# kolenyo2099/revers-o

Hardware: AMD Instinct MI355X
Metric: images/sec embed+top-k (PE-L14-336, 1M x 1024 gallery) (higher is better)
Workload: dtype bf16

## Files before the change

include/revo.h:

```cpp
#ifndef REVO_H
#define REVO_H
#include <stdint.h>

#ifdef __cplusplus
extern "C" {
#endif

typedef struct revo_vit revo_vit;
typedef struct revo_gallery revo_gallery;

typedef struct revo_vit_cfg {
    int32_t image_size, patch_size, width, layers, heads, mlp_dim, out_dim, pool_heads;
    int32_t use_cls;
    int32_t use_ls;
    float ln_eps, rope_theta;
    int32_t pool_mlp_dim;
} revo_vit_cfg;

typedef struct revo_tensor {
    const char* name;
    const float* data;
    int64_t numel;
} revo_tensor;

// ... 62 lines not shown
int32_t revo_search_estimates(int32_t k);
int32_t revo_search_plan(const revo_gallery* g, int32_t n_queries, int32_t k, int64_t* out4);
int32_t revo_search_candidates(revo_gallery* g, const float* queries, int32_t n_queries, int32_t k, int32_t top_m,
                               uint32_t* bounds, void* stream);
int32_t revo_search_finish(revo_gallery* g, int32_t n_queries, int32_t k, int32_t has_threshold, float threshold,
                           int64_t index_offset, const uint32_t* all_bounds, int32_t parts, int32_t top_m, float* scores,
                           int64_t* indices, int32_t* counts, float* cert, void* stream);
int32_t revo_search_exact(revo_gallery* g, int32_t n, const int32_t* q_idx, const float* need, int32_t k,
                          int32_t has_threshold, float threshold, int64_t index_offset, float* scores, int64_t* indices,
                          int32_t* counts, void* stream);
int32_t revo_search_stats(revo_gallery* g, int32_t* out8, void* stream);
int32_t revo_topk_merge(const float* scores, const int64_t* indices, int32_t parts, int32_t n_queries, int32_t k,
                        int32_t has_threshold, float threshold, float* out_scores, int64_t* out_indices,
                        int32_t* out_counts, void* stream);

int64_t revo_topk_packed_bytes(int32_t n_queries, int32_t k);
int32_t revo_topk_merge_packed(const void* packed, int32_t parts, int32_t n_queries, int32_t k, int32_t has_threshold,
                               float threshold, float* out_scores, int64_t* out_indices, int32_t* out_counts,
                               int32_t* unc_count, int32_t* unc_q, float* unc_need, void* stream);

int32_t revo_op_gemm(int32_t epilogue, const void* a_bf16, int64_t lda, const void* b_bf16, int64_t ldb, int32_t m,
                     int32_t n, int32_t k, void* c, int64_t ldc, const float* bias, const float* gamma, void* stream);
int32_t revo_op_gemm_rope(const void* a_bf16, int64_t lda, const void* b_bf16, int64_t ldb, int32_t m, int32_t n, int32_t k,
                          void* c_bf16, int64_t ldc, const float* bias, const float* cos_sin, int32_t seq,
                          int32_t head_dim, int32_t rope_cols, void* stream);
int32_t revo_op_gemm_resid_ln(const void* a_bf16, int64_t lda, const void* b_bf16, int64_t ldb, int32_t m, int32_t n, int32_t k,
                              float* c, int64_t ldc, const float* bias, const float* gamma, void* xb_bf16, int64_t ldxb,
                              void* stats, int32_t* done, void* xlo_bf16, int32_t x_in_planes, int32_t planes_out, void* stream);
int32_t revo_op_gemm_ln_in(int32_t epilogue, const void* a_bf16, int64_t lda, const void* b_bf16, int64_t ldb, int32_t m, int32_t n,
                           int32_t k, void* c_bf16, int64_t ldc, const float* bias, const float* csum, const void* stats,
                           int32_t parts, float eps, void* tele, void* stream);
int32_t revo_op_gemm_ln_in_rope(const void* a_bf16, int64_t lda, const void* b_bf16, int64_t ldb, int32_t m, int32_t n, int32_t k,
                                void* c_bf16, int64_t ldc, const float* bias, const float* csum, const void* stats, int32_t parts,
                                float eps, const float* cos_sin, int32_t seq, int32_t head_dim, int32_t rope_cols, void* stream);
int32_t revo_op_gemm_resid_norm(const void* a_bf16, int64_t lda, const void* b_bf16, int64_t ldb, int32_t m, int32_t n, int32_t k,
                                float* c, int64_t ldc, const float* bias, const float* gamma, void* ln_out_bf16, int64_t ln_ldo,
                                float eps, int32_t* fused, void* stream);
int32_t revo_probe_mfma(const void* src_bf16, int64_t n_elems, float* sink, int32_t blocks, int32_t iters, void* stream);
int64_t revo_probe_mfma_flops(int32_t blocks, int32_t iters);
int32_t revo_probe_copy(void* dst, const void* src, int64_t bytes, void* stream);
#ifdef REVO_EXPERIMENTS
int32_t revo_vit_set_debug_layers(revo_vit* vit, int32_t n_layers);
int32_t revo_vit_read_residual(revo_vit* vit, int32_t batch, float* dst, void* stream);
int32_t revo_vit_read_tap(revo_vit* vit, int32_t which, int32_t batch, void* dst, void* stream);
int32_t revo_search_set_mode(revo_gallery* g, int32_t mode);
int32_t revo_debug_set_remove_chunk(int64_t rows);
int32_t revo_op_set_phase_groups(int32_t groups);
int32_t revo_op_set_qstores(int32_t on);
int32_t revo_debug_gemm_stamps(void* buf, int32_t items);
int32_t revo_debug_attention_clock(void* buf);
int32_t revo_debug_gemm_forms(int32_t reset);
int32_t revo_op_set_gemm_tile(int32_t tile);
int32_t revo_op_set_variant(int32_t flags);
int32_t revo_op_set_ln_fold(int32_t on);
int32_t revo_op_set_gemm_debug(int32_t flags);
int64_t revo_debug_scan_plan(int32_t Q, int64_t rows, int64_t* out, int32_t cap);
int32_t revo_debug_stream_in_planes(const revo_vit* vit, int32_t batch);
int64_t revo_debug_read_workspace(revo_gallery* g, int64_t offset, int64_t bytes, void* host_dst);
int32_t revo_debug_seed_bounds(revo_gallery* g, const uint32_t* bounds);
int32_t revo_probe_gridbar(int32_t mode, void* ctr_err, void* buf, int32_t n16, int32_t blocks, int32_t threads,
                           int32_t iters, float* sink, void* stamps, void* stream);
int32_t revo_debug_scan_stats(int64_t* out8);
#endif
int32_t revo_op_layernorm(const float* x, int64_t ldx, const float* w, const float* b, float eps, int32_t rows,
                          int32_t width, void* out, int64_t ldo, int32_t out_is_bf16, void* stream);
int32_t revo_op_layernorm_logits(const float* x, int64_t ldx, const float* w, const float* b, float eps, int32_t rows,
                                 int32_t width, float* out, int64_t ldo, const float* qk, const float* ck, int32_t heads,
                                 int32_t seq, float* logits, void* stream);
int32_t revo_op_linear_f32(int32_t epi, const float* A, int64_t lda, const float* Wt, int64_t ldw, const float* bias, int32_t M,
                           int32_t N, int32_t K, float* C, int64_t ldc, void* stream);
int32_t revo_op_pool_rows(const float* x, int64_t ldx, const float* logits, int32_t batch, int32_t seq, int32_t width,
                          int32_t heads, float* u, void* stream);
int32_t revo_op_rope(void* qkv_bf16, int64_t ld, const float* cos_sin, int32_t rows, int32_t seq, int32_t width,
                     int32_t heads, void* stream);
int32_t revo_op_attention(const void* qkv_bf16, int64_t ld, void* out_bf16, int64_t ldo, int32_t batch, int32_t seq,
                          int32_t heads, int32_t head_dim, void* stream);
int32_t revo_op_f32_to_bf16(const float* src, int64_t ld_src, void* dst_bf16, int64_t ld_dst, int64_t rows,
                            int32_t cols, void* stream);

int32_t revo_prof_enable(int32_t on);
int32_t revo_prof_reset(void);
int32_t revo_prof_report(char* buf, int32_t capacity);

typedef struct revo_crop_job {
    const uint8_t* src;
    int32_t height, width;
    int64_t row_stride;
    int32_t x0, y0, x1, y1;
} revo_crop_job;
int32_t revo_preprocess_crop_resize(const revo_crop_job* jobs, int32_t n, int32_t out_size, uint8_t* out, void* stream);

#ifdef __cplusplus
}
#endif
#endif
```

revers-o_amd/_lib.py:

```python
import ctypes as C
import os

_HERE = os.path.dirname(os.path.abspath(__file__))
LIB_PATH = os.path.join(_HERE, "librevo.so")


class RevoError(RuntimeError):
    pass


class VitCfg(C.Structure):
    _fields_ = [(n, C.c_int32) for n in (
        "image_size", "patch_size", "width", "layers", "heads", "mlp_dim", "out_dim", "pool_heads",
        "use_cls", "use_ls")] + [("ln_eps", C.c_float), ("rope_theta", C.c_float), ("pool_mlp_dim", C.c_int32)]


class Tensor(C.Structure):
    _fields_ = [("name", C.c_char_p), ("data", C.c_void_p), ("numel", C.c_int64)]


class CropJob(C.Structure):
    _fields_ = [("src", C.c_void_p), ("height", C.c_int32), ("width", C.c_int32), ("row_stride", C.c_int64),
                ("x0", C.c_int32), ("y0", C.c_int32), ("x1", C.c_int32), ("y1", C.c_int32)]

# ... 29 lines not shown
    "revo_search_mmr": (_i32, [_p, _p, _i32, _i32, _i32, _f32, _i32, _f32, _i64, _p, _p, _p, _p, _p]),
    "revo_search_topk": (_i32, [_p, _p, _i32, _i32, _i32, _f32, _i64, _p, _p, _p, _p]),
    "revo_search_topk_large": (_i32, [_p, _p, _i32, _i32, _i32, _f32, _i64, _p, _p, _p, _p]),
    "revo_search_ksel": (_i32, [_i32]),
    "revo_search_set_total_rows": (_i32, [_p, _i64]),
    "revo_search_set_filter": (_i32, [_p, _p, _i64, _i32, _p]),
    "revo_search_set_groups": (_i32, [_p, _p, _i64, _i32, _p]),
    "revo_search_groups": (_i32, [_p, _p, _i32, _i32, _i32, _i32, _f32, _i64, _p, _p, _p, _p, _p, _p]),
    "revo_search_estimates": (_i32, [_i32]),
    "revo_search_plan": (_i32, [_p, _i32, _i32, C.POINTER(C.c_int64)]),
    "revo_search_candidates": (_i32, [_p, _p, _i32, _i32, _i32, _p, _p]),
    "revo_search_finish": (_i32, [_p, _i32, _i32, _i32, _f32, _i64, _p, _i32, _i32, _p, _p, _p, _p, _p]),
    "revo_search_exact": (_i32, [_p, _i32, _p, _p, _i32, _i32, _f32, _i64, _p, _p, _p, _p]),
    "revo_search_stats": (_i32, [_p, C.POINTER(C.c_int32), _p]),
    "revo_topk_merge": (_i32, [_p, _p, _i32, _i32, _i32, _i32, _f32, _p, _p, _p, _p]),
    "revo_topk_packed_bytes": (_i64, [_i32, _i32]),
    "revo_topk_merge_packed": (_i32, [_p, _i32, _i32, _i32, _i32, _f32, _p, _p, _p, _p, _p, _p, _p]),
    "revo_op_gemm": (_i32, [_i32, _p, _i64, _p, _i64, _i32, _i32, _i32, _p, _i64, _p, _p, _p]),
    "revo_op_gemm_resid_ln": (_i32, [_p, _i64, _p, _i64, _i32, _i32, _i32, _p, _i64, _p, _p, _p, _i64, _p, C.POINTER(C.c_int32), _p, _i32,
                                     _i32, _p]),
    "revo_op_gemm_ln_in": (_i32, [_i32, _p, _i64, _p, _i64, _i32, _i32, _i32, _p, _i64, _p, _p, _p, _i32, _f32, _p, _p]),
    "revo_op_gemm_rope": (_i32, [_p, _i64, _p, _i64, _i32, _i32, _i32, _p, _i64, _p, _p, _i32, _i32, _i32, _p]),
    "revo_op_gemm_ln_in_rope": (_i32, [_p, _i64, _p, _i64, _i32, _i32, _i32, _p, _i64, _p, _p, _p, _i32, _f32, _p, _i32, _i32, _i32,
                                       _p]),
    "revo_op_gemm_resid_norm": (_i32, [_p, _i64, _p, _i64, _i32, _i32, _i32, _p, _i64, _p, _p, _p, _i64, _f32, C.POINTER(C.c_int32),
                                       _p]),
    "revo_op_layernorm": (_i32, [_p, _i64, _p, _p, _f32, _i32, _i32, _p, _i64, _i32, _p]),
    "revo_op_layernorm_logits": (_i32, [_p, _i64, _p, _p, _f32, _i32, _i32, _p, _i64, _p, _p, _i32, _i32, _p, _p]),
    "revo_op_linear_f32": (_i32, [_i32, _p, _i64, _p, _i64, _p, _i32, _i32, _i32, _p, _i64, _p]),
    "revo_op_pool_rows": (_i32, [_p, _i64, _p, _i32, _i32, _i32, _i32, _p, _p]),
    "revo_op_rope": (_i32, [_p, _i64, _p, _i32, _i32, _i32, _i32, _p]),
    "revo_op_attention": (_i32, [_p, _i64, _p, _i64, _i32, _i32, _i32, _i32, _p]),
    "revo_op_f32_to_bf16": (_i32, [_p, _i64, _p, _i64, _i64, _i32, _p]),
    "revo_prof_enable": (_i32, [_i32]),
    "revo_prof_reset": (_i32, []),
    "revo_prof_report": (_i32, [C.c_char_p, _i32]),
    "revo_preprocess_crop_resize": (_i32, [C.POINTER(CropJob), _i32, _i32, _p, _p]),
    "revo_probe_mfma": (_i32, [_p, _i64, _p, _i32, _i32, _p]),
    "revo_probe_mfma_flops": (_i64, [_i32, _i32]),
    "revo_probe_copy": (_i32, [_p, _p, _i64, _p]),
}

EXPERIMENT_SIGNATURES = {
    "revo_vit_set_debug_layers": (_i32, [_p, _i32]),
    "revo_vit_read_residual": (_i32, [_p, _i32, _p, _p]),
    "revo_vit_read_tap": (_i32, [_p, _i32, _i32, _p, _p]),
    "revo_search_set_mode": (_i32, [_p, _i32]),
    "revo_op_set_gemm_tile": (_i32, [_i32]),
    "revo_op_set_phase_groups": (_i32, [_i32]),
    "revo_op_set_qstores": (_i32, [_i32]),
    "revo_debug_gemm_forms": (_i32, [_i32]),
    "revo_debug_gemm_stamps": (_i32, [_p, _i32]),
    "revo_debug_attention_clock": (_i32, [_p]),
    "revo_op_set_variant": (_i32, [_i32]),
    "revo_op_set_ln_fold": (_i32, [_i32]),
    "revo_op_set_gemm_debug": (_i32, [_i32]),
    "revo_debug_scan_stats": (_i32, [C.POINTER(C.c_int64)]),
    "revo_debug_set_remove_chunk": (_i32, [_i64]),
    "revo_debug_seed_bounds": (_i32, [_p, _p]),
    "revo_debug_read_workspace": (_i64, [_p, _i64, _i64, _p]),
    "revo_debug_stream_in_planes": (_i32, [_p, _i32]),
    "revo_probe_gridbar": (_i32, [_i32, _p, _p, _i32, _i32, _i32, _i32, _p, _p, _p]),
    "revo_debug_scan_plan": (_i64, [_i32, _i64, C.POINTER(C.c_int64), _i32]),
}
BASE_SIGNATURES = dict(SIGNATURES)
if os.environ.get("REVO_LIBRARY_PATH"):
    LIB_PATH = os.environ["REVO_LIBRARY_PATH"]
elif os.environ.get("REVO_EXPERIMENTS") == "1":
    LIB_PATH = os.path.join(_HERE, "librevo_exp.so")
if os.environ.get("REVO_EXPERIMENTS") == "1":
    SIGNATURES = dict(SIGNATURES, **EXPERIMENT_SIGNATURES)

_lib = None
_lib_exp = None


def product_is_experiment_build():
    return os.environ.get("REVO_EXPERIMENTS") == "1"


def load_exp():
    global _lib_exp
    if _lib_exp is not None:
        return _lib_exp
    import torch
    path = os.path.join(_HERE, "librevo_exp.so")
    if not os.path.exists(path):
        raise RevoError(f"{path} not found: build it with `make -C revers-o_amd/csrc exp`")
    lib = C.CDLL(path)
    for name, (res, args) in dict(BASE_SIGNATURES, **EXPERIMENT_SIGNATURES).items():
        fn = getattr(lib, name)
        fn.restype = res
        fn.argtypes = args
    _lib_exp = lib
    return lib


def load():
    global _lib
    if _lib is not None:
        return _lib
    import torch
    if not os.path.exists(LIB_PATH):
        raise RevoError(
            f"{LIB_PATH} not found: build it with `python -c 'import __graft_entry__ as g; g.build()'` "
            "(or `make -C revers-o_amd/csrc`).  There is no CPU fallback for the hot path.")
# ... 30 lines not shown
```

revers-o_amd/csrc/api.hip:

```cpp
#include <algorithm>
#include <cmath>
#include <cstdlib>
#include <cstring>
#include <map>
#include <memory>
#include <mutex>
#include <string>
#include <vector>

#include "../../include/revo.h"
#include "api_internal.h"
#include "kernels.h"

static thread_local std::string g_err;
void revo_set_error(const std::string& msg) { g_err = msg; }
extern "C" const char* revo_last_error(void) { return g_err.c_str(); }
extern "C" int32_t revo_version(void) { return 100; }

extern "C" int32_t revo_sync(void* stream) {
    REVO_HIP_CHECK(hipStreamSynchronize((hipStream_t)stream));
    return 0;
}

namespace {
// ... 637 lines not shown
}
extern "C" int32_t revo_op_gemm_rope(const void* a, int64_t lda, const void* b, int64_t ldb, int32_t m, int32_t n,
                                     int32_t k, void* c, int64_t ldc, const float* bias, const float* cos_sin,
                                     int32_t seq, int32_t head_dim, int32_t rope_cols, void* stream) {
    API_BEGIN
    revo::GemmArgs g{};
    g.A = (const bf16_t*)a; g.lda = lda; g.B = (const bf16_t*)b; g.ldb = ldb; g.M = m; g.N = n; g.K = k; g.C = c; g.ldc = ldc;
    g.bias = bias; g.rope_cs = (const float2*)cos_sin; g.rope_S = seq; g.rope_hd = head_dim; g.rope_cols = rope_cols;
    return revo::launch_gemm(revo::EPI_BF16_ROPE, g, (hipStream_t)stream);
    API_END
}
extern "C" int32_t revo_op_gemm_ln_in_rope(const void* a, int64_t lda, const void* b, int64_t ldb, int32_t m, int32_t n, int32_t k,
                                           void* c, int64_t ldc, const float* bias, const float* csum, const void* stats,
                                           int32_t parts, float eps, const float* cos_sin, int32_t seq, int32_t head_dim,
                                           int32_t rope_cols, void* stream) {
    API_BEGIN
    REVO_REQUIRE(a && b && c && csum && stats && cos_sin, "op_gemm_ln_in_rope: null argument");
    revo::GemmArgs g{};
    g.A = (const bf16_t*)a; g.lda = lda; g.B = (const bf16_t*)b; g.ldb = ldb; g.M = m; g.N = n; g.K = k; g.C = c; g.ldc = ldc;
    g.bias = bias; g.rope_cs = (const float2*)cos_sin; g.rope_S = seq; g.rope_hd = head_dim; g.rope_cols = rope_cols;
    g.lnc_stats = (const float2*)stats; g.lnc_parts = parts; g.lnc_c = csum; g.lnc_eps = eps;
    return revo::launch_gemm(revo::EPI_BF16_ROPE, g, (hipStream_t)stream);
    API_END
}
extern "C" int32_t revo_op_gemm_resid_norm(const void* a, int64_t lda, const void* b, int64_t ldb, int32_t m, int32_t n, int32_t k,
                                           float* c, int64_t ldc, const float* bias, const float* gamma, void* ln_out,
                                           int64_t ln_ldo, float eps, int32_t* fused, void* stream) {
    API_BEGIN
    REVO_REQUIRE(a && b && c && ln_out && fused, "op_gemm_resid_norm: null argument");
    constexpr long OP_WS_ELEMS = 16l << 20;
    hipStream_t st = (hipStream_t)stream;
    float* ws = nullptr;
    REVO_HIP_CHECK(hipMallocAsync((void**)&ws, OP_WS_ELEMS * 4, st));
    int flag = 0;
    const LnAfter ln{eps, (bf16_t*)ln_out, ln_ldo, &flag, nullptr, nullptr, nullptr, 0, 0};
    const int rc = gemm("gemm_op", revo::EPI_RESID_F32, (const bf16_t*)a, lda, (const bf16_t*)b, ldb, m, n, k, c, ldc, bias, gamma,
                        st, ws, OP_WS_ELEMS, &ln);
    REVO_HIP_CHECK(hipFreeAsync(ws, st));
    *fused = flag;
    return rc;
    API_END
}
#ifdef REVO_EXPERIMENTS
extern "C" int32_t revo_op_set_variant(int32_t flags) {
    revo::gemm_force_gy((flags >> 4) & 15);
    revo::attention_force_nw((flags >> 8) & 15);
    revo::gemm_set_tail_split(((flags >> 12) & 1) ? 0 : 1);
    revo::gemm_set_persistent(((flags >> 16) & 1) ? 0 : 1);
    revo::gemm_set_splitk(((flags >> 17) & 1) ? 0 : 1);
    revo::gemm_set_min_tiles256(((flags >> 18) & 1) ? 0 : 100);
    revo::gemm_set_ring(((flags >> 19) & 1) ? 0 : 1, 0);
    revo::gemm_set_rows192(((flags >> 3) & 1) ? 0 : 1);
    revo::attention_set_shape16((flags >> 20) & 1);
    return 0;
}
extern "C" int32_t revo_op_set_ln_fold(int32_t on) {
    REVO_REQUIRE(on >= 0 && on <= 2, "set_ln_fold: 0 (LayerNorm kernels), 1 (folded, stream in planes: default) or 2 (folded, fp32 stream + bf16 copy)");
    revo::gemm_set_ln_fold(on);
    return 0;
}
extern "C" int32_t revo_op_set_qstores(int32_t on) {
    revo::gemm_set_qstores(on);
    return 0;
}
extern "C" int32_t revo_op_set_phase_groups(int32_t groups) {
    REVO_REQUIRE(groups >= 0 && groups <= 4, "set_phase_groups: 0 (heuristic), 1 (off) or 2..4");
    revo::gemm_set_phase_groups(groups);
    return 0;
}
extern "C" int32_t revo_debug_attention_clock(void* buf) {
    revo::attention_set_clock_buffer((unsigned long long*)buf);
    return 0;
}
extern "C" int32_t revo_debug_gemm_stamps(void* buf, int32_t items) {
    revo::gemm_set_stamps((unsigned long long*)buf, buf ? items : 0);
    return 0;
}
extern "C" int32_t revo_debug_gemm_forms(int32_t reset) { return (int32_t)revo::gemm_debug_forms(reset); }
extern "C" int32_t revo_op_set_gemm_tile(int32_t tile) {
    REVO_REQUIRE(tile == 0 || tile == 128 || tile == 256, "set_gemm_tile: 0, 128 or 256");
    revo::gemm_force_tile(tile);
    return 0;
}
extern "C" int32_t revo_op_set_gemm_debug(int32_t flags) {
    revo::gemm_set_debug(flags & 3);
    revo::gemm_set_stagger(((flags >> 28) & 15) * 200, 2 + ((flags >> 2) & 3));
    revo::topk_scan256_set_debug(((flags >> 13) & 7) | (((flags >> 20) & 255) << 3));
    return revo_op_set_variant(flags);
}
extern "C" int64_t revo_debug_scan_plan(int32_t Q, int64_t rows, int64_t* out, int32_t cap) {
    if (Q < 1 || rows < 1 || !out || cap < 2) return -1;
    return (int64_t)revo::topk_scan256_plan_dump(Q, (long)rows, (long*)out, cap);
}
extern "C" int32_t revo_debug_stream_in_planes(const revo_vit* v, int32_t batch) {
    if (!v || !v->xlo) return 0;
    const int W = v->cfg.width, Md = v->cfg.mlp_dim, rows = batch * v->S;
    return revo::gemm_ln_planes_enabled() && revo::gemm_resid_folds(rows, W, W, W, W, W) && revo::gemm_resid_folds(rows, W, Md, Md, Md, W);
}
#endif
extern "C" int32_t revo_op_layernorm(const float* x, int64_t ldx, const float* w, const float* b, float eps,
                                     int32_t rows, int32_t width, void* out, int64_t ldo, int32_t out_is_bf16,
                                     void* stream) {
    API_BEGIN
    return revo::launch_layernorm(x, ldx, w, b, eps, rows, width, out, ldo, out_is_bf16, (hipStream_t)stream);
    API_END
}
extern "C" int32_t revo_op_layernorm_logits(const float* x, int64_t ldx, const float* w, const float* b, float eps, int32_t rows,
// ... 43 lines not shown
```

revers-o_amd/csrc/attention.hip:

```cpp
#include "kernels.h"
#include <type_traits>

namespace revo {

template <int OFF>
__device__ __forceinline__ uint64_t att_tr_read(uint32_t lds_addr) {
    uint64_t v;
    asm volatile("ds_read_b64_tr_b16 %0, %1 offset:%2" : "=v"(v) : "v"(lds_addr), "n"(OFF));
    return v;
}
template <int ROWB, int DB, int OFF0>
__device__ __forceinline__ void att_v_issue(uint64_t (&v)[2][DB][2], const uint32_t (&va)[DB]) {
#define ATT_V1(S2, D)                                                          \
    v[S2][D][0] = att_tr_read<OFF0 + (16 * S2) * ROWB>(va[D]);                 \
    v[S2][D][1] = att_tr_read<OFF0 + (16 * S2 + 8) * ROWB>(va[D]);
    ATT_V1(0, 0) ATT_V1(0, 1)
    if constexpr (DB == 3) { ATT_V1(0, 2) }
    ATT_V1(1, 0) ATT_V1(1, 1)
    if constexpr (DB == 3) { ATT_V1(1, 2) }
#undef ATT_V1
}
template <int DB, int LEFT = 0>
__device__ __forceinline__ void att_v_wait(uint64_t (&v)[2][DB][2]) {
    if constexpr (DB == 2) {
        asm volatile("s_waitcnt lgkmcnt(%8)"
                     : "+v"(v[0][0][0]), "+v"(v[0][0][1]), "+v"(v[0][1][0]), "+v"(v[0][1][1]), "+v"(v[1][0][0]),
                       "+v"(v[1][0][1]), "+v"(v[1][1][0]), "+v"(v[1][1][1])
                     : "n"(LEFT));
    } else {
        asm volatile("s_waitcnt lgkmcnt(%12)"
                     : "+v"(v[0][0][0]), "+v"(v[0][0][1]), "+v"(v[0][1][0]), "+v"(v[0][1][1]), "+v"(v[0][2][0]),
                       "+v"(v[0][2][1]), "+v"(v[1][0][0]), "+v"(v[1][0][1]), "+v"(v[1][1][0]), "+v"(v[1][1][1]),
                       "+v"(v[1][2][0]), "+v"(v[1][2][1])
                     : "n"(LEFT));
    }
}
typedef uint32_t att_u32x4 __attribute__((ext_vector_type(4)));
template <int OFF>
__device__ __forceinline__ att_u32x4 att_read_b128(uint32_t lds_addr) {
    att_u32x4 v;
    asm volatile("ds_read_b128 %0, %1 offset:%2" : "=v"(v) : "v"(lds_addr), "n"(OFF));
    return v;
}
template <int LEFT>
__device__ __forceinline__ void att_k_wait(att_u32x4& k) {
    asm volatile("s_waitcnt lgkmcnt(%1)" : "+v"(k) : "n"(LEFT));
}
__device__ __forceinline__ bf16x8 att_v_frag(uint64_t lo, uint64_t hi) {
    typedef uint64_t u64x2 __attribute__((ext_vector_type(2)));
    const u64x2 c = {lo, hi};
    return __builtin_bit_cast(bf16x8, c);
}

struct AttDmaSrc {
    __amdgpu_buffer_rsrc_t rsrc;
};
__device__ __forceinline__ void att_dma_init(AttDmaSrc& src, const void* base, int bytes) {
    src.rsrc = __builtin_amdgcn_make_buffer_rsrc((void*)base, 0, bytes, 0x00020000);
}
__device__ __forceinline__ void att_dma_issue(const AttDmaSrc& src, char* dst, uint32_t voff, uint32_t soff) {
    __builtin_amdgcn_raw_ptr_buffer_load_lds(src.rsrc, (__attribute__((address_space(3))) void*)dst, 16, voff, soff, 0, 0);
}

template <int HD, int NW, int DBG = 0, bool STAG = false>
__global__ __launch_bounds__(NW * 64, (HD == 64 && NW >= 6) ? 4 : 1) void attn_fwd_kernel(const bf16_t* __restrict__ qkv, long ld,
                                                          bf16_t* __restrict__ out, long ldo, int S, int H, float c,
                                                          int q_rot, int k_lo
#ifdef REVO_EXPERIMENTS
                                                          , unsigned long long* clk
#endif
                                                          ) {
    static_assert(HD == 64 || HD == 96, "body attention kernel is built for head_dim 64 (B16, L14) and 96 (G14)");
#ifdef REVO_EXPERIMENTS
    unsigned long long clk_t0 = 0, clk_r0 = 0;
    if (clk) { clk_t0 = __builtin_amdgcn_s_memtime(); clk_r0 = __builtin_amdgcn_s_memrealtime(); }
#endif
    constexpr int dbg = DBG;
    constexpr int KS = HD / 16;
    constexpr int DB = HD / 32;
    constexpr int CH = HD / 8;
    constexpr int ROWB = HD == 64 ? 128 : 256;
    constexpr int TILE = 64 * ROWB;
    constexpr int BUF = 2 * TILE;
    static_assert(!STAG || (HD == 64 && NW == 8), "");
    constexpr int LOOK = HD == 64 ? 2 : 1;
    constexpr int NBUF = LOOK + 1 + (STAG ? 1 : 0);
    constexpr int NI = BUF / 1024;
    constexpr int NPW = (NI + NW - 1) / NW;
    constexpr int NDUMMY = NPW * NW - NI;
    constexpr int LPR = ROWB / 16;
    constexpr int RPI = 64 / LPR;
    __shared__ __attribute__((aligned(16))) char lds[NBUF * BUF + NDUMMY * 1024];

    const int tid = threadIdx.x;
    const int wave = __builtin_amdgcn_readfirstlane(tid >> 6), lane = tid & 63;
    const int r = lane & 31, hh = lane >> 5;
    int bh, qblk;
    {
        const int nq = gridDim.x, nbh = gridDim.y, L = blockIdx.y * nq + blockIdx.x;
        const int full = (nbh / 8) * 8;
        if (L < full * nq) {
            const int xcd = L & 7, slot = L >> 3;
            bh = (slot / nq) * 8 + xcd;
            qblk = slot % nq;
        } else {
            const int r = L - full * nq;
            bh = full + r / nq;
            qblk = r % nq;
        }
    }
    const int b = bh / H, h = bh - b * H;
    const int W = H * HD;
    const long rowbase = (long)b * S;
    const int q0 = qblk * (NW * 32) + wave * 32;
    const bool wave_active = q0 < S;
    const bool row_valid = q0 + r < S;
    const int qpos = row_valid ? q0 + r : S - 1;
    const int qrow = q_rot ? (qpos + 1 < S ? qpos + 1 : 0) : qpos;
    const int qrow_c = qrow;

    const bf16_t* kg = qkv + W + h * HD;
    const bf16_t* vg = qkv + 2 * W + h * HD;

    bf16x8 qf[KS];
    {
        const bf16_t* qp = qkv + (rowbase + qrow_c) * ld + h * HD + 8 * hh;
#pragma unroll
        for (int ks = 0; ks < KS; ++ks) qf[ks] = *(const bf16x8*)(qp + 16 * ks);
    }

    const int nkeys = S - k_lo;
    const int nt = (nkeys + 63) / 64;
    AttDmaSrc dma_src;
    att_dma_init(dma_src, kg + (rowbase + k_lo) * ld, (int)(((long)(nkeys - 1) * ld + W + HD) * 2));
    uint32_t dma_voff[NPW];
#pragma unroll
    for (int i = 0; i < NPW; ++i) {
        const int j = wave + NW * i;
        const int row = j * RPI + lane / LPR;
        const int cp = lane % LPR;
        const int isv = row >= 64, key = row & 63;
        const int swz = HD == 64 ? (isv ? (((key >> 1) & 1) << 2) : ((key >> 1) & 7))
                                 : (isv ? ((key & 3) << 2) : (key & 15));
        const int ch = cp ^ swz;
        dma_voff[i] = (ch < CH && j < NI) ? (uint32_t)(((long)key * ld + (isv ? W : 0)) * 2 + ch * 16) : 0x80000000u;
// ... 165 lines not shown
            ps2 = (f32x2){1.f, 1.f};
            _Pragma("unroll") for (int kb_ = 0; kb_ < 2; ++kb_)
                _Pragma("unroll") for (int j_ = 0; j_ < 8; ++j_) pw[kb_][j_] = pack_bf16x2(sacc[kb_][2 * j_], sacc[kb_][2 * j_ + 1]);
        }
        float ps = ps2.x + ps2.y;
        if (!__all(ps < 0x1p80f)) {
            asm volatile("" ::: "memory");
            scores();
            float mx = -INFINITY;
#pragma unroll
            for (int kblk = 0; kblk < 2; ++kblk)
#pragma unroll
                for (int i = 0; i < 16; ++i) mx = fmaxf(mx, sacc[kblk][i]);
            mx = fmaxf(mx, __shfl_xor(mx, 32, 64)) * c;
            const float m_new = fmaxf(m_run, mx);
            const float alpha = __builtin_amdgcn_exp2f(m_run - m_new);
            m_run = m_new;
            l_run *= alpha;
#pragma unroll
            for (int d = 0; d < DB; ++d)
#pragma unroll
                for (int i = 0; i < 16; ++i) oacc[d][i] *= alpha;
            exps();
            ps = ps2.x + ps2.y;
        }
        l_run += ps;
        if (!(STAG && late)) pv_tile(std::integral_constant<int, SB>{}, true);
    };
#ifdef REVO_ATTN_PRIO
    if (REVO_ATTN_PRIO == 1 ? wave >= NW / 2 : wave < NW / 2) __builtin_amdgcn_s_setprio(1);
#endif
    for (int t = 0; t < nt; t += NBUF) {
        tile_step(std::integral_constant<int, 0>{}, t);
        if (NBUF > 1 && t + 1 < nt) tile_step(std::integral_constant<int, 1 % NBUF>{}, t + 1);
        if (NBUF > 2 && t + 2 < nt) tile_step(std::integral_constant<int, 2 % NBUF>{}, t + 2);
        if (NBUF > 3 && t + 3 < nt) tile_step(std::integral_constant<int, 3 % NBUF>{}, t + 3);
    }
    if constexpr (STAG) {
        if (late && wave_active && nt > 0) {
            switch ((nt - 1) % NBUF) {
                case 0: pv_tile(std::integral_constant<int, 0>{}, false); break;
                case 1: pv_tile(std::integral_constant<int, BUF>{}, false); break;
                case 2: pv_tile(std::integral_constant<int, 2 * BUF>{}, false); break;
                default: pv_tile(std::integral_constant<int, 3 * BUF>{}, false); break;
            }
        }
    }

    if constexpr (HD == 64) {
        __builtin_amdgcn_s_barrier();
        if (wave_active) {
            constexpr int RS = 144;
            char* slab = lds + wave * (32 * RS);
            const float l_tot = l_run + __shfl_xor(l_run, 32, 64);
            const float inv = 1.0f / l_tot;
#pragma unroll
            for (int d = 0; d < DB; ++d)
#pragma unroll
                for (int g = 0; g < 4; ++g) {
                    uint2 o;
                    o.x = pack_bf16x2(oacc[d][4 * g + 0] * inv, oacc[d][4 * g + 1] * inv);
                    o.y = pack_bf16x2(oacc[d][4 * g + 2] * inv, oacc[d][4 * g + 3] * inv);
                    *(uint2*)(slab + r * RS + (d * 32 + 8 * g + 4 * hh) * 2) = o;
                }
#pragma unroll
            for (int it = 0; it < 4; ++it) {
                const int rl = it * 8 + (lane >> 3);
                const uint4 v = *(const uint4*)(slab + rl * RS + (lane & 7) * 16);
                const int qp = q0 + rl;
                if (qp < S) {
                    const int qr = q_rot ? (qp + 1 < S ? qp + 1 : 0) : qp;
                    *(uint4*)(out + (rowbase + qr) * ldo + h * HD + (lane & 7) * 8) = v;
                }
            }
        }
    } else if (wave_active) {
        const float l_tot = l_run + __shfl_xor(l_run, 32, 64);
        if (row_valid) {
            const float inv = 1.0f / l_tot;
            bf16_t* op = out + (rowbase + qrow) * ldo + h * HD;
#pragma unroll
            for (int d = 0; d < DB; ++d)
#pragma unroll
                for (int g = 0; g < 4; ++g) {
                    uint2 o;
                    o.x = pack_bf16x2(oacc[d][4 * g + 0] * inv, oacc[d][4 * g + 1] * inv);
                    o.y = pack_bf16x2(oacc[d][4 * g + 2] * inv, oacc[d][4 * g + 3] * inv);
                    *(uint2*)(op + d * 32 + 8 * g + 4 * hh) = o;
                }
        }
    }
#undef ATT_ISSUE_TILE
#undef ATT_WAIT_TILE
#ifdef REVO_EXPERIMENTS
    if (clk && threadIdx.x == 0) {
        const unsigned long long t1 = __builtin_amdgcn_s_memtime(), r1 = __builtin_amdgcn_s_memrealtime();
        unsigned long long* dst = clk + 2 * ((size_t)blockIdx.y * gridDim.x + blockIdx.x);
        dst[0] = t1 - clk_t0;
        dst[1] = r1 - clk_r0;
    }
#endif
}



__device__ __forceinline__ void att16_mfma(f32x4& acc, const bf16x8& a, const bf16x8& b) {
// ... 275 lines not shown
        if (t + 2 < nt) tile_step(std::integral_constant<int, 2>{}, t + 2);
    }

    att16_mfma_settle();
    __builtin_amdgcn_s_barrier();
    if (wave_active) {
        constexpr int RS = 144;
        char* slab = lds + wave * (32 * RS);
#pragma unroll
        for (int nb = 0; nb < 2; ++nb) {
            float l_tot = l_run[nb] + __shfl_xor(l_run[nb], 16, 64);
            l_tot += __shfl_xor(l_tot, 32, 64);
            const float inv = 1.0f / l_tot;
#pragma unroll
            for (int d = 0; d < 4; ++d) {
                uint2 o;
                o.x = pack_bf16x2(oacc[d][nb][0] * inv, oacc[d][nb][1] * inv);
                o.y = pack_bf16x2(oacc[d][nb][2] * inv, oacc[d][nb][3] * inv);
                *(uint2*)(slab + (nb * 16 + li) * RS + (d * 16 + 4 * lq) * 2) = o;
            }
        }
#pragma unroll
        for (int it = 0; it < 4; ++it) {
            const int rl = it * 8 + (lane >> 3);
            const uint4 v = *(const uint4*)(slab + rl * RS + (lane & 7) * 16);
            const int qp = q0 + rl;
            if (qp < S) {
                const int qr = q_rot ? (qp + 1 < S ? qp + 1 : 0) : qp;
                *(uint4*)(out + (rowbase + qr) * ldo + h * HD + (lane & 7) * 8) = v;
            }
        }
    }
#undef ATT_ISSUE_TILE
#undef ATT_WAIT_TILE
#ifdef REVO_EXPERIMENTS
    if (clk && threadIdx.x == 0) {
        const unsigned long long t1 = __builtin_amdgcn_s_memtime(), r1 = __builtin_amdgcn_s_memrealtime();
        unsigned long long* dst = clk + 2 * ((size_t)blockIdx.y * gridDim.x + blockIdx.x);
        dst[0] = t1 - clk_t0;
        dst[1] = r1 - clk_r0;
    }
#endif
}

#ifdef REVO_EXPERIMENTS
static unsigned long long* g_attn_clk = nullptr;
void attention_set_clock_buffer(unsigned long long* buf) { g_attn_clk = buf; }
#define ATT_CLK_ARG , g_attn_clk
#else
#define ATT_CLK_ARG
#endif
static int g_attn_shape16 = 0;
void attention_set_shape16(int on) { g_attn_shape16 = on; }
template <int HD, int NW>
static void launch_attn_nw(const bf16_t* qkv, long ld, bf16_t* out, long ldo, int B, int S, int H, float c, int q_rot,
                           int k_lo, hipStream_t st) {
    const int rows = S;
    dim3 grid((rows + NW * 32 - 1) / (NW * 32), B * H), block(NW * 64);
#ifdef REVO_EXPERIMENTS
    if constexpr (HD == 64 && NW == 8) {
        if (getenv("REVO_ATTN_STAG")) {
            hipLaunchKernelGGL((attn_fwd_kernel<HD, NW, 0, true>), grid, block, 0, st, qkv, ld, out, ldo, S, H, c, q_rot, k_lo ATT_CLK_ARG);
            return;
        }
        if (const char* e = getenv("REVO_ATTN_DBG")) {
            switch (atoi(e)) {
#define ATT_DBG_CASE(D) case D: hipLaunchKernelGGL((attn_fwd_kernel<HD, NW, D>), grid, block, 0, st, qkv, ld, out, ldo, S, H, c, q_rot, k_lo ATT_CLK_ARG); return;
                ATT_DBG_CASE(1) ATT_DBG_CASE(2) ATT_DBG_CASE(3) ATT_DBG_CASE(4) ATT_DBG_CASE(7) ATT_DBG_CASE(8) ATT_DBG_CASE(16)
                ATT_DBG_CASE(24) ATT_DBG_CASE(28) ATT_DBG_CASE(31) ATT_DBG_CASE(32) ATT_DBG_CASE(64) ATT_DBG_CASE(96)
#undef ATT_DBG_CASE
                default: break;
            }
        }
    }
#endif
#ifdef REVO_EXPERIMENTS
    if constexpr (HD == 64) {
        if (g_attn_shape16) {
            if constexpr (NW == 8) {
                if (const char* e = getenv("REVO_ATTN16_DBG")) {
                    switch (atoi(e)) {
                        case 1: hipLaunchKernelGGL((attn16_fwd_kernel<NW, 1>), grid, block, 0, st, qkv, ld, out, ldo, S, H, c, q_rot, k_lo ATT_CLK_ARG); return;
                        case 2: hipLaunchKernelGGL((attn16_fwd_kernel<NW, 2>), grid, block, 0, st, qkv, ld, out, ldo, S, H, c, q_rot, k_lo ATT_CLK_ARG); return;
                        case 3: hipLaunchKernelGGL((attn16_fwd_kernel<NW, 3>), grid, block, 0, st, qkv, ld, out, ldo, S, H, c, q_rot, k_lo ATT_CLK_ARG); return;
                        default: break;
                    }
                }
            }
            hipLaunchKernelGGL((attn16_fwd_kernel<NW>), grid, block, 0, st, qkv, ld, out, ldo, S, H, c, q_rot, k_lo ATT_CLK_ARG);
            return;
        }
    }
#endif
    hipLaunchKernelGGL((attn_fwd_kernel<HD, NW>), grid, block, 0, st, qkv, ld, out, ldo, S, H, c, q_rot, k_lo ATT_CLK_ARG);
}

static int g_attn_force_nw = 0;
void attention_force_nw(int nw) { g_attn_force_nw = nw; }
int launch_attention_ex(const bf16_t* qkv, long ld, bf16_t* out, long ldo, int B, int S, int H, int hd, int has_cls,
                        hipStream_t st) {
    REVO_REQUIRE(hd == 64 || hd == 96, "attention: head_dim must be 64 (PE-Core B16 / L14) or 96 (G14)");
    REVO_REQUIRE(ld % 8 == 0 && ldo % 4 == 0, "attention: strides must keep 16-byte alignment");
    if (B <= 0 || S <= 0) return 0;
    const float scale = 1.0f / sqrtf((float)hd);
    const float c = scale * 1.44269504088896340736f;
    const int lo = (has_cls && S > 1 && (S - 1 + 63) / 64 < (S + 63) / 64) ? 1 : 0;
    const int rows = S;
    int best = 4, best_blocks = 1 << 30;
    for (int nw : {8, 7, 6, 4}) {
        const int blocks = (rows + nw * 32 - 1) / (nw * 32);
        if (blocks < best_blocks) { best_blocks = blocks; best = nw; }
    }
    if (g_attn_force_nw) best = g_attn_force_nw;
    if (hd == 64) {
        switch (best) {
            case 8: launch_attn_nw<64, 8>(qkv, ld, out, ldo, B, S, H, c, lo, lo, st); break;
            case 7: launch_attn_nw<64, 7>(qkv, ld, out, ldo, B, S, H, c, lo, lo, st); break;
            case 6: launch_attn_nw<64, 6>(qkv, ld, out, ldo, B, S, H, c, lo, lo, st); break;
            default: launch_attn_nw<64, 4>(qkv, ld, out, ldo, B, S, H, c, lo, lo, st); break;
        }
    } else {
        if (best >= 6) launch_attn_nw<96, 8>(qkv, ld, out, ldo, B, S, H, c, lo, lo, st);
        else launch_attn_nw<96, 4>(qkv, ld, out, ldo, B, S, H, c, lo, lo, st);
    }
    REVO_HIP_CHECK(hipGetLastError());
    return 0;
}
int launch_attention(const bf16_t* qkv, long ld, bf16_t* out, long ldo, int B, int S, int H, int hd, hipStream_t st) {
    return launch_attention_ex(qkv, ld, out, ldo, B, S, H, hd, 1, st);
}


}
```

revers-o_amd/csrc/kernels.h:

```cpp
#pragma once
#include "common.h"

namespace revo {

enum GemmEpi {
    EPI_BF16 = 0,
    EPI_BF16_GELU = 1,
    EPI_RESID_F32 = 2,
    EPI_F32 = 3,
    EPI_PATCH = 4,
    EPI_BF16_ROPE = 5,
};

struct GemmArgs {
    const bf16_t* A; long lda;
    const bf16_t* B; long ldb;
    int M, N, K;
    void* C; long ldc;
    const float* bias;
    const float* gamma;
    const float* pos;
    int S, G2, cls;
    int gy;
    const float2* rope_cs;
// ... 39 lines not shown
unsigned gemm_debug_forms(int reset);
#endif
int launch_gemm_f32_ring(const GemmArgs& a, hipStream_t st);
bool gemm_resid_folds(int M, int N, int K, long lda, long ldb, long ldc);
int launch_planes_to_f32(const bf16_t* hi, const bf16_t* lo, long ldp, float* x, long ldx, long rows, int W, hipStream_t st);
#ifdef REVO_EXPERIMENTS
void gemm_set_debug(int d);
void gemm_set_stagger(int cycles, int groups);
void gemm_set_stamps(unsigned long long* buf, int items);
void gemm_set_phase_groups(int g);
#endif
void gemm_force_gy(int gy);
void gemm_set_tail_split(int on);
void gemm_force_tile(int t);

constexpr int LN_MAXH = 16;
struct LnLogits { const float* qk; const float* ck; float* logits; int H, S; };
int launch_layernorm(const float* x, long ldx, const float* w, const float* b, float eps, int rows, int W,
                     void* out, long ldo, int out_is_bf16, hipStream_t st, const LnLogits* logits = nullptr);
int launch_fold_ln_linear(const float* w, const float* gamma, const float* beta, const float* bias, int rows, int cols,
                          bf16_t* out, long ld, float* csum, float* bias_out, hipStream_t st);
int launch_patchify(const void* images, int is_u8, int B, int img, int P, bf16_t* out, long Kp, hipStream_t st);
int launch_probe_qk(const float* q, const float* Wk, const float* bk, int W, int heads, float* qk, float* ck, hipStream_t st);
int launch_pool_head_rows(const float* x, long ldx, int B, int S, int W, int H, const float* logits, float* u, hipStream_t st);
int launch_gemm_f32_skinny(int epi, const float* A, long lda, long a_group_stride, int group_cols, const float* Wt, long ldw,
                           const float* bias, int M, int N, int K, float* C, long ldc, hipStream_t st);
int launch_transpose_f32(const float* src, int rows, int cols, float* dst, hipStream_t st);
int launch_split_hi_lo_hi(const float* src, long rows, int cols, float scale, bf16_t* dst, long ld, hipStream_t st);
int launch_cls_rows(float* x, long ldx, const float* cls, const float* pos, int B, int S, int W, hipStream_t st);
int launch_rope(bf16_t* qkv, long ld, const float2* cs, int rows, int S, int W, int heads, hipStream_t st);
int launch_f32_to_bf16(const float* src, long ld_src, bf16_t* dst, long ld_dst, long rows, int cols, hipStream_t st);
int launch_l2norm_rows(const float* src, long ld_src, float* dst_f32, long ld_f32, bf16_t* dst_bf16, long ld_bf16,
                       long rows, int D, hipStream_t st, int normalize = 1, float* row_stats = nullptr,
                       uint32_t* max_stats = nullptr, uint32_t* zero_a = nullptr, long zero_a_words = 0,
                       uint32_t* zero_b = nullptr, long zero_b_words = 0, const long long* dst_rows = nullptr);

constexpr long REMOVE_MAX_CHUNK = 65536;
int launch_remove_count(const uint32_t* bits, long N, long chunk, uint32_t* cnt, uint32_t* first, hipStream_t st);
int launch_remove_gather(const uint32_t* bits, long N, long row0, long len, long j0, const uint4* src, uint4* dst,
                         int u4_per_row, hipStream_t st);

int launch_attention(const bf16_t* qkv, long ld, bf16_t* out, long ldo, int B, int S, int H, int hd, hipStream_t st);
int launch_attention_ex(const bf16_t* qkv, long ld, bf16_t* out, long ldo, int B, int S, int H, int hd, int has_cls,
                        hipStream_t st);
void gemm_set_min_tiles256(int n);
void gemm_set_ring(int on, int max_tiles);
void gemm_set_splitk(int on);
void gemm_set_persistent(int on);
void gemm_set_qstores(int on);
void gemm_set_rows192(int on);
void gemm_set_ln_fold(int on);
bool gemm_ln_planes_enabled();
void attention_force_nw(int nw);
void attention_set_shape16(int on);
#ifdef REVO_EXPERIMENTS
void attention_set_clock_buffer(unsigned long long* buf);
#endif

struct ScanArgs {
    const bf16_t* Qb; long ldq;
    const bf16_t* Gb; long ldg;
    int Q; long N; int D;
    int ksel;
    int splits;
    uint64_t* part;
    const uint32_t* allow;
};
int topk_scan_workspace_splits(int Q, long N);
int launch_topk_scan(const ScanArgs& a, hipStream_t st);
int launch_topk_reduce(uint64_t* part, int Q, int splits, int ksel, hipStream_t st);
constexpr int EXACT_COL_CAP = 2048;
constexpr int EXACT_L3_SLICES = 32;
static_assert(EXACT_L3_SLICES * 64 == EXACT_COL_CAP, "the brute-force partial lists live in the collect buffer");
enum ExactCtr : int {
    CTR_UNCERTIFIED,
    CTR_BRUTEFORCE,
    CTR_CHECKED,
    CTR_COLLECTED,
    CTR_MODE3_FAILED,
    CTR_FROM_SEGS,
    CTR_GROUPED,
    CTR_LARGE_FALLBACK,
    CTR_PAIR_PASSES,
    CTR_SLOTS
};
struct ExactWs {
    int* ctr;
    int* unc_q;
    float* unc_lb;
    bf16_t* qb_u;
    long ldqb;
    int* col_cnt;
    uint64_t* col;
    int* over_j;
    int* orow;
    int cap;
};
constexpr int GROUP_K1 = 50;
struct GroupWs {
    const int* group_of_row;
    int* gq;
    int* chosen;
    int hits;
    int has_thr; float thr;
};
struct GroupOut {
// ... 278 lines not shown
```

Baseline: 2423.

## Choose attention waves and ring depth from measured occupancy per device

Replaces the fixed rule that picked the attention kernel's waves per workgroup by fewest blocks with a planner. The planner queries CU count and resident blocks per instantiation and picks the plan with the fewest scheduling rounds, falling back to the fewest-blocks choice unless the gain passes a one-eighth margin. It adds a shallower ring (one tile of lookahead) variant for 4-wave hd=64, and raises the launch-bounds occupancy hint to 4 for all hd=64 variants, which may constrain registers for the 4-wave kernel. It also adds a debug API to report the chosen plan and a flag to force the ring depth.

```diff
diff --git a/include/revo.h b/include/revo.h
--- a/include/revo.h
+++ b/include/revo.h
@@ -138,6 +138,7 @@
 int32_t revo_debug_gemm_forms(int32_t reset);
 int32_t revo_op_set_gemm_tile(int32_t tile);
 int32_t revo_op_set_variant(int32_t flags);
+int32_t revo_debug_attention_plan(int32_t batch, int32_t seq, int32_t heads, int32_t head_dim, int32_t* out4);
 int32_t revo_op_set_ln_fold(int32_t on);
 int32_t revo_op_set_gemm_debug(int32_t flags);
 int64_t revo_debug_scan_plan(int32_t Q, int64_t rows, int64_t* out, int32_t cap);
diff --git a/revers-o_amd/_lib.py b/revers-o_amd/_lib.py
--- a/revers-o_amd/_lib.py
+++ b/revers-o_amd/_lib.py
@@ -105,6 +105,7 @@
     "revo_debug_gemm_forms": (_i32, [_i32]),
     "revo_debug_gemm_stamps": (_i32, [_p, _i32]),
     "revo_debug_attention_clock": (_i32, [_p]),
+    "revo_debug_attention_plan": (_i32, [_i32, _i32, _i32, _i32, _p]),
     "revo_op_set_variant": (_i32, [_i32]),
     "revo_op_set_ln_fold": (_i32, [_i32]),
     "revo_op_set_gemm_debug": (_i32, [_i32]),
diff --git a/revers-o_amd/csrc/api.hip b/revers-o_amd/csrc/api.hip
--- a/revers-o_amd/csrc/api.hip
+++ b/revers-o_amd/csrc/api.hip
@@ -713,7 +713,13 @@
     revo::gemm_set_ring(((flags >> 19) & 1) ? 0 : 1, 0);
     revo::gemm_set_rows192(((flags >> 3) & 1) ? 0 : 1);
     revo::attention_set_shape16((flags >> 20) & 1);
-    return 0;
+    revo::attention_force_ring((flags >> 21) & 3);
+    return 0;
+}
+extern "C" int32_t revo_debug_attention_plan(int32_t batch, int32_t seq, int32_t heads, int32_t head_dim, int32_t* out4) {
+    API_BEGIN
+    return revo::attention_plan(batch, seq, heads, head_dim, out4);
+    API_END
 }
 extern "C" int32_t revo_op_set_ln_fold(int32_t on) {
     REVO_REQUIRE(on >= 0 && on <= 2, "set_ln_fold: 0 (LayerNorm kernels), 1 (folded, stream in planes: default) or 2 (folded, fp32 stream + bf16 copy)");
diff --git a/revers-o_amd/csrc/attention.hip b/revers-o_amd/csrc/attention.hip
--- a/revers-o_amd/csrc/attention.hip
+++ b/revers-o_amd/csrc/attention.hip
@@ -1,5 +1,8 @@
 #include "kernels.h"
+#include <algorithm>
+#include <mutex>
 #include <type_traits>
+#pragma clang diagnostic ignored "-Wpass-failed"
 
 namespace revo {
 
@@ -62,8 +65,8 @@
     __builtin_amdgcn_raw_ptr_buffer_load_lds(src.rsrc, (__attribute__((address_space(3))) void*)dst, 16, voff, soff, 0, 0);
 }
 
-template <int HD, int NW, int DBG = 0, bool STAG = false>
-__global__ __launch_bounds__(NW * 64, (HD == 64 && NW >= 6) ? 4 : 1) void attn_fwd_kernel(const bf16_t* __restrict__ qkv, long ld,
+template <int HD, int NW, int DBG = 0, bool STAG = false, int LOOK_ = (HD == 64 ? 2 : 1)>
+__global__ __launch_bounds__(NW * 64, HD == 64 ? 4 : 1) void attn_fwd_kernel(const bf16_t* __restrict__ qkv, long ld,
                                                           bf16_t* __restrict__ out, long ldo, int S, int H, float c,
                                                           int q_rot, int k_lo
 #ifdef REVO_EXPERIMENTS
@@ -83,7 +86,9 @@
     constexpr int TILE = 64 * ROWB;
     constexpr int BUF = 2 * TILE;
     static_assert(!STAG || (HD == 64 && NW == 8), "");
-    constexpr int LOOK = HD == 64 ? 2 : 1;
+    static_assert(LOOK_ == 1 || LOOK_ == 2, "ATT_WAIT_TILE counts at most one tile in flight behind the awaited one");
+    static_assert(!STAG || LOOK_ == 2, "the staggered experiment keeps its own depth: four slots");
+    constexpr int LOOK = LOOK_;
     constexpr int NBUF = LOOK + 1 + (STAG ? 1 : 0);
     constexpr int NI = BUF / 1024;
     constexpr int NPW = (NI + NW - 1) / NW;
@@ -91,6 +96,8 @@
     constexpr int LPR = ROWB / 16;
     constexpr int RPI = 64 / LPR;
     __shared__ __attribute__((aligned(16))) char lds[NBUF * BUF + NDUMMY * 1024];
+    static_assert(HD != 64 || NW * 32 * 144 <= NBUF * BUF, "the epilogue's wave-private slabs (32 rows of 144 bytes per wave) reuse the ring");
+    static_assert(NBUF * BUF + NDUMMY * 1024 <= 64 * 1024, "LDS per workgroup");
 
     const int tid = threadIdx.x;
     const int wave = __builtin_amdgcn_readfirstlane(tid >> 6), lane = tid & 63;
@@ -362,6 +369,8 @@
         if (wave_active) {
             constexpr int RS = 144;
             char* slab = lds + wave * (32 * RS);
+            const int lane = NPW > 2 ? (int)__builtin_amdgcn_mbcnt_hi(~0u, __builtin_amdgcn_mbcnt_lo(~0u, 0u)) : (tid & 63);
+            const int r = lane & 31, hh = lane >> 5;
             const float l_tot = l_run + __shfl_xor(l_run, 32, 64);
             const float inv = 1.0f / l_tot;
 #pragma unroll
@@ -743,13 +752,13 @@
 #endif
 static int g_attn_shape16 = 0;
 void attention_set_shape16(int on) { g_attn_shape16 = on; }
-template <int HD, int NW>
+template <int HD, int NW, int LOOK = (HD == 64 ? 2 : 1)>
 static void launch_attn_nw(const bf16_t* qkv, long ld, bf16_t* out, long ldo, int B, int S, int H, float c, int q_rot,
                            int k_lo, hipStream_t st) {
     const int rows = S;
     dim3 grid((rows + NW * 32 - 1) / (NW * 32), B * H), block(NW * 64);
 #ifdef REVO_EXPERIMENTS
-    if constexpr (HD == 64 && NW == 8) {
+    if constexpr (HD == 64 && NW == 8 && LOOK == 2) {
         if (getenv("REVO_ATTN_STAG")) {
             hipLaunchKernelGGL((attn_fwd_kernel<HD, NW, 0, true>), grid, block, 0, st, qkv, ld, out, ldo, S, H, c, q_rot, k_lo ATT_CLK_ARG);
             return;
@@ -766,7 +775,7 @@
     }
 #endif
 #ifdef REVO_EXPERIMENTS
-    if constexpr (HD == 64) {
+    if constexpr (HD == 64 && LOOK == 2) {
         if (g_attn_shape16) {
             if constexpr (NW == 8) {
                 if (const char* e = getenv("REVO_ATTN16_DBG")) {
@@ -783,11 +792,87 @@
         }
     }
 #endif
-    hipLaunchKernelGGL((attn_fwd_kernel<HD, NW>), grid, block, 0, st, qkv, ld, out, ldo, S, H, c, q_rot, k_lo ATT_CLK_ARG);
-}
-
+    hipLaunchKernelGGL((attn_fwd_kernel<HD, NW, 0, false, LOOK>), grid, block, 0, st, qkv, ld, out, ldo, S, H, c, q_rot, k_lo ATT_CLK_ARG);
+}
+
+struct AttnPlan {
+    int hd, waves, ring;
+    const void* kernel;
+    bool planned;
+};
+constexpr int ATTN_ROUNDS_MARGIN_DEN = 8;
+static const AttnPlan g_attn_plans[] = {
+    {64, 8, 3, (const void*)attn_fwd_kernel<64, 8, 0, false, 2>, true}, {64, 7, 3, (const void*)attn_fwd_kernel<64, 7, 0, false, 2>, true},
+    {64, 6, 3, (const void*)attn_fwd_kernel<64, 6, 0, false, 2>, true},
+    {64, 5, 3, (const void*)attn_fwd_kernel<64, 5, 0, false, 2>, false},
+    {64, 4, 3, (const void*)attn_fwd_kernel<64, 4, 0, false, 2>, true}, {64, 4, 2, (const void*)attn_fwd_kernel<64, 4, 0, false, 1>, true},
+    {96, 8, 2, (const void*)attn_fwd_kernel<96, 8, 0, false, 1>, true}, {96, 4, 2, (const void*)attn_fwd_kernel<96, 4, 0, false, 1>, true},
+};
+constexpr int ATTN_NPLANS = (int)(sizeof(g_attn_plans) / sizeof(g_attn_plans[0]));
+struct AttnDeviceInfo {
+    int cus = 0;
+    int resident[ATTN_NPLANS] = {};
+};
+static AttnDeviceInfo g_attn_dev[REVO_MAX_DEVICES];
+static std::mutex g_attn_dev_mutex;
+static int attn_device_info(AttnDeviceInfo& info) {
+    int dev = 0;
+    REVO_HIP_CHECK(hipGetDevice(&dev));
+    REVO_REQUIRE(dev >= 0 && dev < REVO_MAX_DEVICES, "attention: device ordinal out of range");
+    std::lock_guard<std::mutex> lock(g_attn_dev_mutex);
+    AttnDeviceInfo& d = g_attn_dev[dev];
+    if (d.cus == 0) {
+        int cus = 0;
+        REVO_HIP_CHECK(hipDeviceGetAttribute(&cus, hipDeviceAttributeMultiprocessorCount, dev));
+        REVO_REQUIRE(cus > 0, "attention: the device reports no compute units");
+        for (int i = 0; i < ATTN_NPLANS; ++i) {
+            int n = 0;
+            REVO_HIP_CHECK(hipOccupancyMaxActiveBlocksPerMultiprocessor(&n, g_attn_plans[i].kernel, g_attn_plans[i].waves * 64, 0));
+            REVO_REQUIRE(n > 0, "attention: a kernel instantiation does not fit a compute unit");
+            d.resident[i] = n;
+        }
+        d.cus = cus;
+    }
+    info = d;
+    return 0;
+}
 static int g_attn_force_nw = 0;
+static int g_attn_force_ring = 0;
 void attention_force_nw(int nw) { g_attn_force_nw = nw; }
+void attention_force_ring(int ring) { g_attn_force_ring = ring; }
+static int attn_choose_plan(int B, int S, int H, int hd, int* blocks_out, int* resident_out) {
+    AttnDeviceInfo info;
+    if (const int rc = attn_device_info(info)) return rc;
+    int forced_nw = g_attn_force_nw;
+    if (forced_nw && hd == 96) forced_nw = forced_nw >= 6 ? 8 : 4;
+    const int forced_ring = hd == 64 ? (g_attn_force_ring == 1 ? 2 : g_attn_force_ring == 2 ? 3 : forced_nw ? 3 : 0) : 0;
+    int best = -1, best_blocks = 0, base = -1, base_blocks = 0;
+    double best_rounds = 0, base_rounds = 0;
+    for (int i = 0; i < ATTN_NPLANS; ++i) {
+        const AttnPlan& p = g_attn_plans[i];
+        if (p.hd != hd || (forced_nw && p.waves != forced_nw) || (forced_ring && p.ring != forced_ring)) continue;
+        const int blocks = (S + p.waves * 32 - 1) / (p.waves * 32);
+        if (!p.planned && !forced_nw) continue;
+        const double rounds = std::max(1.0, (double)B * H * blocks / ((double)info.cus * info.resident[i]));
+        if (best < 0 || rounds < best_rounds || (rounds == best_rounds && blocks < best_blocks)) {
+            best = i; best_blocks = blocks; best_rounds = rounds;
+        }
+        if (base < 0 || blocks < base_blocks) { base = i; base_blocks = blocks; base_rounds = rounds; }
+    }
+    REVO_REQUIRE(best >= 0, "attention: no kernel is built for the forced waves per workgroup and ring depth");
+    if (best_rounds * ATTN_ROUNDS_MARGIN_DEN >= base_rounds * (ATTN_ROUNDS_MARGIN_DEN - 1)) { best = base; best_blocks = base_blocks; }
+    if (blocks_out) *blocks_out = best_blocks;
+    if (resident_out) *resident_out = info.resident[best];
+    return best;
+}
+int attention_plan(int B, int S, int H, int hd, int out[4]) {
+    REVO_REQUIRE(out && B >= 1 && S >= 1 && H >= 1 && (hd == 64 || hd == 96), "attention_plan: bad arguments");
+    int blocks = 0, resident = 0;
+    const int i = attn_choose_plan(B, S, H, hd, &blocks, &resident);
+    if (i < 0) return i;
+    out[0] = g_attn_plans[i].waves; out[1] = g_attn_plans[i].ring; out[2] = blocks; out[3] = resident;
+    return 0;
+}
 int launch_attention_ex(const bf16_t* qkv, long ld, bf16_t* out, long ldo, int B, int S, int H, int hd, int has_cls,
                         hipStream_t st) {
     REVO_REQUIRE(hd == 64 || hd == 96, "attention: head_dim must be 64 (PE-Core B16 / L14) or 96 (G14)");
@@ -796,22 +881,21 @@
     const float scale = 1.0f / sqrtf((float)hd);
     const float c = scale * 1.44269504088896340736f;
     const int lo = (has_cls && S > 1 && (S - 1 + 63) / 64 < (S + 63) / 64) ? 1 : 0;
-    const int rows = S;
-    int best = 4, best_blocks = 1 << 30;
-    for (int nw : {8, 7, 6, 4}) {
-        const int blocks = (rows + nw * 32 - 1) / (nw * 32);
-        if (blocks < best_blocks) { best_blocks = blocks; best = nw; }
-    }
-    if (g_attn_force_nw) best = g_attn_force_nw;
+    const int plan = attn_choose_plan(B, S, H, hd, nullptr, nullptr);
+    if (plan < 0) return plan;
+    const AttnPlan& p = g_attn_plans[plan];
     if (hd == 64) {
-        switch (best) {
-            case 8: launch_attn_nw<64, 8>(qkv, ld, out, ldo, B, S, H, c, lo, lo, st); break;
-            case 7: launch_attn_nw<64, 7>(qkv, ld, out, ldo, B, S, H, c, lo, lo, st); break;
-            case 6: launch_attn_nw<64, 6>(qkv, ld, out, ldo, B, S, H, c, lo, lo, st); break;
-            default: launch_attn_nw<64, 4>(qkv, ld, out, ldo, B, S, H, c, lo, lo, st); break;
+        switch (p.waves * 10 + p.ring) {
+            case 83: launch_attn_nw<64, 8>(qkv, ld, out, ldo, B, S, H, c, lo, lo, st); break;
+            case 73: launch_attn_nw<64, 7>(qkv, ld, out, ldo, B, S, H, c, lo, lo, st); break;
+            case 63: launch_attn_nw<64, 6>(qkv, ld, out, ldo, B, S, H, c, lo, lo, st); break;
+            case 53: launch_attn_nw<64, 5>(qkv, ld, out, ldo, B, S, H, c, lo, lo, st); break;
+            case 43: launch_attn_nw<64, 4>(qkv, ld, out, ldo, B, S, H, c, lo, lo, st); break;
+            case 42: launch_attn_nw<64, 4, 1>(qkv, ld, out, ldo, B, S, H, c, lo, lo, st); break;
+            default: REVO_REQUIRE(false, "attention: plan without a launch");
         }
     } else {
-        if (best >= 6) launch_attn_nw<96, 8>(qkv, ld, out, ldo, B, S, H, c, lo, lo, st);
+        if (p.waves == 8) launch_attn_nw<96, 8>(qkv, ld, out, ldo, B, S, H, c, lo, lo, st);
         else launch_attn_nw<96, 4>(qkv, ld, out, ldo, B, S, H, c, lo, lo, st);
     }
     REVO_HIP_CHECK(hipGetLastError());
diff --git a/revers-o_amd/csrc/kernels.h b/revers-o_amd/csrc/kernels.h
--- a/revers-o_amd/csrc/kernels.h
+++ b/revers-o_amd/csrc/kernels.h
@@ -115,6 +115,8 @@
 void gemm_set_ln_fold(int on);
 bool gemm_ln_planes_enabled();
 void attention_force_nw(int nw);
+void attention_force_ring(int ring);
+int attention_plan(int B, int S, int H, int hd, int out[4]);
 void attention_set_shape16(int on);
 #ifdef REVO_EXPERIMENTS
 void attention_set_clock_buffer(unsigned long long* buf);
```

After: 2445, median of 6. Within noise of the previous version (+0.9%).
